# Guillaume-SOULIER/SOS-Radiative-Transfer

Measured on AMD Instinct MI355X. Metric: SOS columns/sec to 1e-4 convergence (Ntau=200, Nmu=128), higher is better.
Workload: dtype f64

## Files before the change

### sos-radiative-transfer_amd/csrc/jn_gemm.hip

```cpp
#include "jn_gemm_tile.hpp"

namespace sosrt {

namespace {

#ifndef SOSRT_DENSE_SLAB_RT
#define SOSRT_DENSE_SLAB_RT 1
#endif
constexpr int DENSE_SLAB_RT = SOSRT_DENSE_SLAB_RT;
#ifndef SOSRT_LIVE_TILE_MAJOR
#define SOSRT_LIVE_TILE_MAJOR 1
#endif
constexpr int DENSE_SLAB_ROWS = 16 * DENSE_SLAB_RT;

__device__ __forceinline__ void write_live_list(const GemmArgs& g) {
    __shared__ int s_cnt[4];
    const int tid = threadIdx.x, lane = tid & 63, wave = tid >> 6;
    int before = 0;
    for (int base = 0; base < g.B; base += 256) {
        const bool f = base + tid < g.B && g.active[g.col0 + base + tid] != 0;
        const unsigned long long mk = __ballot(f);
        if (lane == 0) s_cnt[wave] = __popcll(mk);
        __syncthreads();
        int pre = before, tot = 0;
        for (int w = 0; w < 4; ++w) {
            if (w < wave) pre += s_cnt[w];
            tot += s_cnt[w];
        }
        const int at = pre + __popcll(mk & ((1ull << lane) - 1));
        if (f && at < g.live_cap) g.live_list[at] = base + tid;
        before += tot;
        __syncthreads();
    }
    for (int i = before + tid; i < g.live_cap; i += 256) g.live_list[i] = -1;
}

template <bool SYM, bool ATM>
__device__ __forceinline__ void jn_gemm_dense(const GemmArgs& g, const AtmSets& at) {
    if (g.live_list && blockIdx.x == gridDim.x - 1) {
        write_live_list(g);
        return;
    }
    publish_live(g);
    __shared__ double sA[(SYM ? 2 : 1) * 16 * (GEMM_RT > 2 ? GEMM_RT : 2) * A_LD];
    __shared__ double sB[GEMM_KC * B_LD];
    __shared__ int s_any;
    const int tiles_main = (g.n_main + 16 * GEMM_RT - 1) / (16 * GEMM_RT);
    const int tiles_slab = (g.n_slab + DENSE_SLAB_ROWS - 1) / DENSE_SLAB_ROWS;
    const int tiles = tiles_main + tiles_slab;
    const int nct = (g.D + GEMM_BN - 1) / GEMM_BN;
    const int id = blockIdx.x;
    int tile = (id / (8 * nct)) * 8 + (id & 7);
    const int bn0 = ((id >> 3) % nct) * GEMM_BN;
    if (tile >= tiles) return;
    if (ATM || g.lr_rank >= 0) {
        if (tile >= tiles_slab) {
            lowrank_tile<false, ListRows, ATM>(g, ListRows{g.rows_main, g.n_main}, tile - tiles_slab, 16 * GEMM_RT, bn0, true, at);
            return;
        }
        tile += tiles_main;
    }
    if (tile < tiles_main) {
        gemm_tile<GEMM_RT, false, false, SYM>(g, sA, sB, &s_any, tile, bn0, ListRows{g.rows_main, g.n_main}, true);
    } else if (g.Wmix && g.slab_tile_group) {
        const int st = tile - tiles_main;
        gemm_tile<DENSE_SLAB_RT, false, false, SYM>(g, sA, sB, &s_any, st, bn0, ListRows{g.rows_slab, g.n_slab}, true,
                                                    g.Wmix + (size_t)g.slab_tile_group[st * DENSE_SLAB_ROWS / 32] * g.Dp * g.Wld);
    } else if (g.slab_tile_group) {
        const int st = tile - tiles_main;
        GemmArgs gs = g;
        gs.Wr = g.Wr + (size_t)g.slab_tile_group[st * DENSE_SLAB_ROWS / 32] * g.Dp * g.Wld;
        gemm_tile<DENSE_SLAB_RT, true, false, SYM>(gs, sA, sB, &s_any, st, bn0, ListRows{g.rows_slab, g.n_slab}, true);
    } else {
        gemm_tile<DENSE_SLAB_RT, true, false, SYM>(g, sA, sB, &s_any, tile - tiles_main, bn0, ListRows{g.rows_slab, g.n_slab}, true);
    }
}
template <bool SYM>
__global__ __launch_bounds__(256, GEMM_WPS) void k_jn_gemm(GemmArgs g) { jn_gemm_dense<SYM, false>(g, AtmSets()); }
__global__ __launch_bounds__(256, GEMM_WPS) void k_jn_gemm_atm(GemmArgs g, AtmSets at) { jn_gemm_dense<true, true>(g, at); }

template <int RT, bool DEEP, bool SYM, bool ATM = false>
__device__ __forceinline__ void gemm_live_columns(const GemmArgs& g, double* sA, double* sB, const AtmSets& at = AtmSets()) {
    __shared__ int s_w[4];
    __shared__ int s_col;
    const int tid = threadIdx.x, lane = tid & 63, wave = tid >> 6;
    const int ts = (g.max_slab + 16 * TAIL_RT_SLAB - 1) / (16 * TAIL_RT_SLAB);
    const int tm = (g.max_main + 16 * RT - 1) / (16 * RT);
    const int nct = (g.D + GEMM_BN - 1) / GEMM_BN;
    const int id = blockIdx.x;
    const int xq = (id / (8 * nct)) * 8 + (id & 7), bn0 = ((id >> 3) % nct) * GEMM_BN;
// ... 13 lines not shown
        if (lane == 0) s_w[wave] = __popcll(mk);
        __syncthreads();
        int pre = before, tot = 0;
        for (int w = 0; w < 4; ++w) {
            if (w < wave) pre += s_w[w];
            tot += s_w[w];
        }
        if (f && pre + __popcll(mk & ((2ull << lane) - 1)) == ci + 1) s_col = g.col0 + base + tid;
        before += tot;
        __syncthreads();
        if (before > ci) break;
    }
    const int b = s_col;
    if (g.live_list && xq < (SOSRT_LIVE_TILE_MAJOR ? (g.live_cap > 0 ? g.live_cap : 1) : 1 << 30) &&
        (SOSRT_LIVE_TILE_MAJOR || tt == 0) && bn0 == 0 && tid == 0 && ci < g.live_cap)
        g.live_list[ci] = b < 0 ? -1 : b - g.col0;
    if (b < 0) return;
    const int iu = g.idx_up ? g.idx_up[b] : 0;
    const int ns = g.idx_up ? g.idx_down[b] - iu + 1 : 0;
    if (tt < ts) {
        if (tt * 16 * TAIL_RT_SLAB >= ns) return;
        if (g.Wmix)
            gemm_tile<TAIL_RT_SLAB, false, DEEP, SYM>(g, sA, sB, nullptr, tt, bn0, ColumnRows{b * g.L, iu, ns, ns, true},
                                                      false, g.Wmix + (size_t)g.mix_group[b] * g.Dp * g.Wld);
        else if (g.mix_group) {
            GemmArgs gs = g;
            gs.Wr = g.Wr + (size_t)g.mix_group[b] * g.Dp * g.Wld;
            gemm_tile<TAIL_RT_SLAB, true, DEEP, SYM>(gs, sA, sB, nullptr, tt, bn0, ColumnRows{b * g.L, iu, ns, ns, true}, false);
        } else
            gemm_tile<TAIL_RT_SLAB, true, DEEP, SYM>(g, sA, sB, nullptr, tt, bn0, ColumnRows{b * g.L, iu, ns, ns, true}, false);
    } else {
        const int t2 = tt - ts;
        if (t2 * 16 * RT >= g.L - ns) return;
        if (ATM || g.lr_rank >= 0) lowrank_tile<false, ColumnRows, ATM>(g, ColumnRows{b * g.L, iu, ns, g.L - ns, false}, t2, 16 * RT, bn0, false, at);
        else gemm_tile<RT, false, DEEP, SYM>(g, sA, sB, nullptr, t2, bn0, ColumnRows{b * g.L, iu, ns, g.L - ns, false}, false);
    }
}

template <bool SYM>
__global__ __launch_bounds__(256, SYM ? 4 : GEMM_WPS) void k_jn_gemm_cols(GemmArgs g) {
    publish_live(g);
    __shared__ double sA[(SYM ? 2 : 1) * 16 * GEMM_RT * A_LD];
    __shared__ double sB[GEMM_KC * B_LD];
    gemm_live_columns<GEMM_RT, false, SYM>(g, sA, sB);
}
__global__ __launch_bounds__(256, 4) void k_jn_gemm_cols_atm(GemmArgs g, AtmSets at) {
    publish_live(g);
    __shared__ double sA[2 * 16 * GEMM_RT * A_LD];
    __shared__ double sB[GEMM_KC * B_LD];
    gemm_live_columns<GEMM_RT, false, true, true>(g, sA, sB, at);
}
constexpr bool kTailDeepSym = false;
constexpr int kTailWpsSym = 4;
template <bool SYM>
__global__ __launch_bounds__(256, SYM ? kTailWpsSym : 2) void k_jn_gemm_tail(GemmArgs g) {
    publish_live(g);
    __shared__ double sA[(SYM ? 2 : 1) * 16 * TAIL_RT * A_LD];
    __shared__ double sB[GEMM_KC * B_LD];
    gemm_live_columns<TAIL_RT, SYM ? kTailDeepSym : true, SYM>(g, sA, sB);
}
__global__ __launch_bounds__(256, kTailWpsSym) void k_jn_gemm_tail_atm(GemmArgs g, AtmSets at) {
    publish_live(g);
    __shared__ double sA[2 * 16 * TAIL_RT * A_LD];
    __shared__ double sB[GEMM_KC * B_LD];
    gemm_live_columns<TAIL_RT, kTailDeepSym, true, true>(g, sA, sB, at);
}
constexpr int kTailDeepCols = 32;
__global__ __launch_bounds__(256, 2) void k_jn_gemm_tail_deep(GemmArgs g) {
    publish_live(g);
    __shared__ double sA[2 * 16 * TAIL_RT * A_LD];
    __shared__ double sB[GEMM_KC * B_LD];
    gemm_live_columns<TAIL_RT, true, true>(g, sA, sB);
}
__global__ __launch_bounds__(256, 2) void k_jn_gemm_tail_deep_atm(GemmArgs g, AtmSets at) {
    publish_live(g);
    __shared__ double sA[2 * 16 * TAIL_RT * A_LD];
    __shared__ double sB[GEMM_KC * B_LD];
    gemm_live_columns<TAIL_RT, true, true, true>(g, sA, sB, at);
}

template <bool ATM>
__device__ __forceinline__ void jn_gemm_lone(const GemmArgs& g, const AtmSets& at) {
    extern __shared__ __attribute__((aligned(16))) double s_lone[];
    __shared__ int s_w[4];
    __shared__ int s_col[4];
    const int tid = threadIdx.x, lane = tid & 63, wave = tid >> 6;
    if (blockIdx.x == gridDim.x - 1) {
        if (g.host_pub && tid == 0) publish_live_now(g);
        return;
    }
    const int ts = (g.max_slab + 15) / 16, tm = (g.max_main + 15) / 16;
    const int nct = (g.D + GEMM_BN - 1) / GEMM_BN;
    const int id = blockIdx.x;
    const int xq = (id / (8 * nct)) * 8 + (id & 7), bn0 = ((id >> 3) % nct) * GEMM_BN;
    const int cap = g.live_cap > 0 ? g.live_cap : 1;
    const int tq = xq / cap, ci = xq % cap;
    if (tq >= ts + tm) return;
    const int tt = (ATM || g.lr_rank >= 0) ? tq : (tq < tm ? ts + tq : tq - tm);
    int fl = 0, iu_c = 0, id_c = -1, mg_c = 0;
    if (tid < g.B) {
        const int c = g.col0 + tid;
        fl = g.active[c];
        if (g.idx_up) {
            iu_c = g.idx_up[c]; id_c = g.idx_down[c];
            if (g.mix_group) mg_c = g.mix_group[c];
        }
    }
    LoneFrag f0, f1;
    const int nkb = (g.Ks >> 2) / LONE_KB;
    if (!ATM && tt >= ts && g.lr_rank < 0) {
// ... 14 lines not shown
            if (w < wave) pre += s_w[w];
            tot += s_w[w];
        }
        if (f && pre + __popcll(mk & ((2ull << lane) - 1)) == ci + 1) {
            s_col[0] = g.col0 + base + tid; s_col[1] = iu_c; s_col[2] = id_c - iu_c + 1; s_col[3] = mg_c;
        }
        before += tot;
        __syncthreads();
        if (before > ci || base + 256 >= g.B) break;
        fl = 0;
        if (base + 256 + tid < g.B) {
            const int c = g.col0 + base + 256 + tid;
            fl = g.active[c];
            if (g.idx_up) {
                iu_c = g.idx_up[c]; id_c = g.idx_down[c];
                if (g.mix_group) mg_c = g.mix_group[c];
            }
        }
    }
    const int b = s_col[0];
    if (g.live_list && tq == 0 && bn0 == 0 && tid == 0 && ci < g.live_cap) g.live_list[ci] = b < 0 ? -1 : b - g.col0;
    if (b < 0) return;
    const int iu = g.idx_up ? s_col[1] : 0, ns = g.idx_up ? s_col[2] : 0, mg = s_col[3];
    if (tt < ts) {
        if (tt * 16 >= ns) return;
        if (g.Wmix) gemm_tile_lone<false, false>(g, s_lone, tt, bn0, ColumnRows{b * g.L, iu, ns, ns, true}, f0, f1, g.Wmix + (size_t)mg * g.Dp * g.Wld);
        else if (g.mix_group) {
            GemmArgs gs = g;
            gs.Wr = g.Wr + (size_t)mg * g.Dp * g.Wld;
            gemm_tile_lone<true, false>(gs, s_lone, tt, bn0, ColumnRows{b * g.L, iu, ns, ns, true}, f0, f1);
        } else gemm_tile_lone<true, false>(g, s_lone, tt, bn0, ColumnRows{b * g.L, iu, ns, ns, true}, f0, f1);
    } else {
        if ((tt - ts) * 16 >= g.L - ns) return;
        if (ATM || g.lr_rank >= 0) lowrank_tile<false, ColumnRows, ATM>(g, ColumnRows{b * g.L, iu, ns, g.L - ns, false}, tt - ts, 16, bn0, false, at);
        else gemm_tile_lone<false, true>(g, s_lone, tt - ts, bn0, ColumnRows{b * g.L, iu, ns, g.L - ns, false}, f0, f1);
    }
}
__global__ __launch_bounds__(256, 1) void k_jn_gemm_lone(GemmArgs g) { jn_gemm_lone<false>(g, AtmSets()); }
__global__ __launch_bounds__(256, 1) void k_jn_gemm_lone_atm(GemmArgs g, AtmSets at) { jn_gemm_lone<true>(g, at); }

}

void launch_gemm_tail(hipStream_t s, const GemmArgs& a, int cols, bool small_tiles, bool regs, const AtmSets* at) {
    if (regs && a.sym) {
        const int ts = (a.max_slab + 15) / 16, tm = (a.max_main + 15) / 16;
        if (cols <= 0 || ts + tm <= 0) return;
        const int nct = (a.D + GEMM_BN - 1) / GEMM_BN;
        const int lds = 16 * (a.D + 2) * 8;
        static PerDeviceOnce big_lds;
        if (big_lds.first()) {
            hipFuncSetAttribute(reinterpret_cast<const void*>(k_jn_gemm_lone), hipFuncAttributeMaxDynamicSharedMemorySize, 150 * 1024);
            hipFuncSetAttribute(reinterpret_cast<const void*>(k_jn_gemm_lone_atm), hipFuncAttributeMaxDynamicSharedMemorySize, 150 * 1024);
        }
        const dim3 lgrid((unsigned)((cols * (ts + tm) + 7) / 8 * 8 * nct + 1));
        if (at) hipLaunchKernelGGL(k_jn_gemm_lone_atm, lgrid, dim3(256), (size_t)lds, s, a, *at);
        else hipLaunchKernelGGL(k_jn_gemm_lone, lgrid, dim3(256), (size_t)lds, s, a);
        return;
    }
    const int rt = small_tiles ? TAIL_RT : GEMM_RT;
    const int ts = (a.max_slab + 16 * TAIL_RT_SLAB - 1) / (16 * TAIL_RT_SLAB);
    const int tm = (a.max_main + 16 * rt - 1) / (16 * rt);
    if (cols <= 0 || ts + tm <= 0) return;
    const int nct = (a.D + GEMM_BN - 1) / GEMM_BN;
    dim3 grid((unsigned)((cols * (ts + tm) + 7) / 8 * 8 * nct));
    if (at) {
        if (small_tiles && cols <= kTailDeepCols) hipLaunchKernelGGL(k_jn_gemm_tail_deep_atm, grid, dim3(256), 0, s, a, *at);
        else if (small_tiles) hipLaunchKernelGGL(k_jn_gemm_tail_atm, grid, dim3(256), 0, s, a, *at);
// ... 69 lines not shown
                                                        double* __restrict__ out) {
    __shared__ double s_w[4], s_a[4];
    __shared__ int s_nan[4];
    const int q = blockIdx.y, tid = threadIdx.x;
    const double* Wq = W + (size_t)q * per;
    double wmax = 0, amax = 0;
    int nan = 0;
    const size_t n = (size_t)D * D;
    for (size_t e = (size_t)blockIdx.x * 256 + tid; e < n; e += (size_t)gridDim.x * 256) {
        const int k = (int)(e / D), m = (int)(e % D);
        const double x = Wq[(size_t)k * Wld + m], y = Wq[(size_t)(D - 1 - k) * Wld + (D - 1 - m)];
        const double ax = fabs(x), d = fabs(x - y);
        nan |= (ax != ax) || (d != d);
        wmax = fmax(wmax, ax); amax = fmax(amax, d);
    }
#pragma unroll
    for (int o = 32; o > 0; o >>= 1) {
        wmax = fmax(wmax, __shfl_xor(wmax, o, 64)); amax = fmax(amax, __shfl_xor(amax, o, 64));
        nan |= __shfl_xor(nan, o, 64);
    }
    if ((tid & 63) == 0) { s_w[tid >> 6] = wmax; s_a[tid >> 6] = amax; s_nan[tid >> 6] = nan; }
    __syncthreads();
    if (tid == 0) {
        for (int i = 1; i < 4; ++i) { wmax = fmax(wmax, s_w[i]); amax = fmax(amax, s_a[i]); nan |= s_nan[i]; }
        double* o = out + ((size_t)q * gridDim.x + blockIdx.x) * 2;
        o[0] = nan ? __builtin_nan("") : wmax;
        o[1] = nan ? __builtin_nan("") : amax;
    }
}
void launch_fold_asymmetry(hipStream_t s, int S, int nblk, int D, int Wld, size_t per, const double* W, double* out) {
    hipLaunchKernelGGL(k_fold_asymmetry, dim3((unsigned)nblk, (unsigned)S), dim3(256), 0, s, D, Wld, per, W, out);
}

void launch_gemm(hipStream_t s, const GemmArgs& a, const AtmSets* at) {
    const int tiles = (a.n_main + 16 * GEMM_RT - 1) / (16 * GEMM_RT) + (a.n_slab + DENSE_SLAB_ROWS - 1) / DENSE_SLAB_ROWS;
    if (tiles <= 0) return;
    const int nct = (a.D + GEMM_BN - 1) / GEMM_BN;
    dim3 grid((unsigned)((tiles + 7) / 8 * 8 * nct + (a.live_list ? 1 : 0)));
    if (at) hipLaunchKernelGGL(k_jn_gemm_atm, grid, dim3(256), (size_t)a.pad_lds, s, a, *at);
    else if (a.sym) hipLaunchKernelGGL(k_jn_gemm<true>, grid, dim3(256), (size_t)a.pad_lds, s, a);
    else hipLaunchKernelGGL(k_jn_gemm<false>, grid, dim3(256), (size_t)a.pad_lds, s, a);
}

__global__ void k_symfold(int nmat, int N, int D, int Dp, int Wld, const double* __restrict__ W, double* __restrict__ SA) {
    const size_t per = (size_t)Dp * Wld;
    const size_t i = (size_t)blockIdx.x * blockDim.x + threadIdx.x;
    if (i >= per * nmat) return;
    const size_t mat = i / per, r = i % per;
    const int k = (int)(r / Wld), c = (int)(r % Wld), Nh = Wld >> 1;
    const int m = c < Nh ? c : c - Nh;
    double out = 0.0;
    if (k < N && m < N) {
        const double* w = W + mat * per;
        const double p = w[(size_t)k * Wld + m], pf = w[(size_t)(D - 1 - k) * Wld + (D - 1 - m)];
        const double q = w[(size_t)(D - 1 - k) * Wld + m], qf = w[(size_t)k * Wld + (D - 1 - m)];
        out = c < Nh ? 0.25 * ((p + pf) + (q + qf)) : 0.25 * ((p + pf) - (q + qf));
    }
    SA[i] = out;
}
void launch_symfold(hipStream_t s, int nmat, int N, int D, int Dp, int Wld, const double* W, double* SA) {
    const size_t n = (size_t)Dp * Wld * nmat;
    hipLaunchKernelGGL(k_symfold, dim3((unsigned)((n + 255) / 256)), dim3(256), 0, s, nmat, N, D, Dp, Wld, W, SA);
}

}
```

### sos-radiative-transfer_amd/csrc/jn_gemm_tile.hpp

```cpp
#pragma once
#include "kernels.hpp"
#include "transport_util.hpp"

namespace sosrt {

namespace {

typedef double f64x4 __attribute__((ext_vector_type(4)));

constexpr int A_LD = GEMM_KC + 2;
constexpr int B_LD = GEMM_BN + 16;

struct ListRows {
    const int* rows;
    int n;
    __device__ int operator()(int lr) const { return lr < n ? (rows ? rows[lr] : lr) : -1; }
};
struct ColumnRows {
    int base, iu, ns, n;
    bool slab;
    __device__ int operator()(int lr) const {
        if (lr >= n) return -1;
        return base + (slab ? iu + lr : (lr < iu ? lr : lr + ns));
    }
// ... 310 lines not shown
        const double cf_ = pass_ ? cf_r : cf_a;                                                                   \
        const int k0_ = 4 * (b_ - pass_ * nkb) * LONE_KB + fk;                                                    \
        _Pragma("unroll") for (int q = 0; q < LONE_KB; ++q) {                                                     \
            const int k_ = k0_ + 4 * q;                                                                           \
            const bool ok_ = grow >= 0 && k_ < Nn;                                                                \
            const double a_ = arow[k_], m_ = arow[D - 1 - k_];                  \
            const double u_ = ok_ ? cf_ * (a_ + m_) : 0.0, v_ = ok_ ? cf_ * (a_ - m_) : 0.0;                      \
            accx = __builtin_amdgcn_mfma_f64_16x16x4f64(u_, F.s[q], accx, 0, 0, 0);                               \
            accy = __builtin_amdgcn_mfma_f64_16x16x4f64(v_, F.a[q], accy, 0, 0, 0);                               \
        }                                                                                                         \
    }
    for (int blk = 0; blk < nblk; blk += 2) {
        SOSRT_LONE_COMPUTE(f0, blk);
        SOSRT_LONE_LOAD(f0, blk + 2);
        if (blk + 1 < nblk) {
            SOSRT_LONE_COMPUTE(f1, blk + 1);
            SOSRT_LONE_LOAD(f1, blk + 3);
        }
    }
#undef SOSRT_LONE_LOAD
#undef SOSRT_LONE_COMPUTE
#pragma unroll
    for (int r = 0; r < 4; ++r) {
        const int gr = row_of(tile * 16 + 4 * r + fk);
        if (gr >= 0 && mcol < Nn) {
            const double x = accx[r], y = accy[r];
            g.C[(size_t)gr * D + mcol] = x + y;
            g.C[(size_t)gr * D + D - 1 - mcol] = x - y;
        }
    }
}

constexpr int LR_ROWS = 4;
template <bool COH, bool ATM = false>
__device__ __forceinline__ void lowrank_rows(const GemmArgs& g, const int (&rows)[LR_ROWS], int lane, const AtmSets& at = AtmSets()) {
    const int D = g.D, R = g.lr_rank;
    __amdgpu_buffer_rsrc_t rA[LR_ROWS], rC[LR_ROWS];
    double cf[LR_ROWS];
    int Ri[LR_ROWS];
    const double* __restrict__ Ui[LR_ROWS];
    const double* __restrict__ Vi[LR_ROWS];
#pragma unroll
    for (int i = 0; i < LR_ROWS; ++i) {
        const int r = rows[i] >= 0 ? rows[i] : rows[0];
        const int bytes = rows[i] >= 0 ? D * 8 : 0;
        rA[i] = make_rsrc(g.A + (size_t)r * D, bytes);
        rC[i] = make_rsrc(g.C + (size_t)r * D, bytes);
        cf[i] = rows[i] >= 0 ? g.ca[rows[i]] : 0.0;
        if constexpr (ATM) {
            const int st = __builtin_amdgcn_readfirstlane(at.col_atm[r / g.L]);
            Ri[i] = __builtin_amdgcn_readfirstlane(at.lr_ranks[st]);
            Ui[i] = g.lrU + (size_t)st * kLowRankMax * D;
            Vi[i] = g.lrV + (size_t)st * kLowRankMax * D;
        }
    }
    const double* __restrict__ U = g.lrU;
    const double* __restrict__ V = g.lrV;
    double m[LR_ROWS][kLowRankMax];
#pragma unroll
    for (int i = 0; i < LR_ROWS; ++i)
#pragma unroll
        for (int q = 0; q < kLowRankMax; ++q) m[i][q] = 0.0;
#pragma unroll 2
    for (int k = 2 * lane; k < D; k += 128) {
        double2 x[LR_ROWS];
#pragma unroll
        for (int i = 0; i < LR_ROWS; ++i) x[i] = bload2_aux<COH ? 16 : 0>(rA[i], k * 8, 0);
#pragma unroll
        for (int q = 0; q < kLowRankMax; ++q) {
            if constexpr (ATM) {
#pragma unroll
                for (int i = 0; i < LR_ROWS; ++i)
                    if (q < Ri[i]) {
                        const double2 u = *reinterpret_cast<const double2*>(Ui[i] + (size_t)q * D + k);
                        m[i][q] = __builtin_fma(x[i].y, u.y, __builtin_fma(x[i].x, u.x, m[i][q]));
                    }
            } else if (q < R) {
                const double2 u = *reinterpret_cast<const double2*>(U + (size_t)q * D + k);
#pragma unroll
                for (int i = 0; i < LR_ROWS; ++i) m[i][q] = __builtin_fma(x[i].y, u.y, __builtin_fma(x[i].x, u.x, m[i][q]));
            }
        }
    }
#pragma unroll
    for (int s = 32; s >= 1; s >>= 1)
#pragma unroll
        for (int q = 0; q < kLowRankMax; ++q) {
            if constexpr (ATM) {
#pragma unroll
                for (int i = 0; i < LR_ROWS; ++i)
                    if (q < Ri[i]) m[i][q] += __shfl_xor(m[i][q], s);
            } else if (q < R) {
#pragma unroll
                for (int i = 0; i < LR_ROWS; ++i) m[i][q] += __shfl_xor(m[i][q], s);
            }
        }
    if constexpr (!COH && !ATM) {
        if (g.mom) {
#pragma unroll
            for (int i = 0; i < LR_ROWS; ++i) {
                const int r = rows[i] >= 0 ? rows[i] : rows[0];
                const __amdgpu_buffer_rsrc_t rM = make_rsrc(g.mom + (size_t)r * kMomDoubles, rows[i] >= 0 ? kMomDoubles * 8 : 0);
                const double x = lane == 0 ? m[i][0] : (lane == 1 ? m[i][2] : (lane == 2 ? cf[i] : 0.0));
                const double y = lane == 0 ? m[i][1] : (lane == 1 ? m[i][3] : 0.0);
                bstore2(rM, lane * 16, 0, make_double2(x, y));
            }
            return;
        }
    }
#pragma unroll 2
    for (int k = 2 * lane; k < D; k += 128) {
        if constexpr (ATM) {
            double2 o[LR_ROWS];
#pragma unroll
            for (int i = 0; i < LR_ROWS; ++i) o[i] = make_double2(0.0, 0.0);
#pragma unroll
            for (int q = 0; q < kLowRankMax; ++q) {
#pragma unroll
                for (int i = 0; i < LR_ROWS; ++i)
                    if (q < Ri[i]) {
                        const double2 v = *reinterpret_cast<const double2*>(Vi[i] + (size_t)q * D + k);
                        o[i].x = __builtin_fma(m[i][q], v.x, o[i].x);
                        o[i].y = __builtin_fma(m[i][q], v.y, o[i].y);
                    }
            }
#pragma unroll
            for (int i = 0; i < LR_ROWS; ++i) bstore2_aux<COH ? 17 : 0>(rC[i], k * 8, 0, make_double2(cf[i] * o[i].x, cf[i] * o[i].y));
        } else {
            double vx[kLowRankMax], vy[kLowRankMax];
#pragma unroll
            for (int q = 0; q < kLowRankMax; ++q) {
                vx[q] = 0.0; vy[q] = 0.0;
                if (q < R) {
                    const double2 v = *reinterpret_cast<const double2*>(V + (size_t)q * D + k);
                    vx[q] = v.x; vy[q] = v.y;
                }
            }
#pragma unroll
            for (int i = 0; i < LR_ROWS; ++i)
                bstore2_aux<COH ? 17 : 0>(rC[i], k * 8, 0, make_double2(lr_expand(m[i], vx, R, cf[i]), lr_expand(m[i], vy, R, cf[i])));
        }
    }
}
template <bool COH, class RowOf, bool ATM = false>
__device__ __forceinline__ void lowrank_tile(const GemmArgs& g, RowOf row_of, int tile, int BM, int bn0, bool check_active,
                                             const AtmSets& at = AtmSets()) {
    const int nct = (g.D + GEMM_BN - 1) / GEMM_BN, ct = bn0 / GEMM_BN;
    const int lane = threadIdx.x & 63, wave = __builtin_amdgcn_readfirstlane(threadIdx.x) >> 6;
    const int per = (BM - ct + nct - 1) / nct;
    const bool chk = check_active && g.active && g.check_tiles;
    for (int j = LR_ROWS * wave; j < per; j += 4 * LR_ROWS) {
        int rows[LR_ROWS];
        int n = 0;
#pragma unroll
        for (int i = 0; i < LR_ROWS; ++i) {
            int r = j + i < per ? __builtin_amdgcn_readfirstlane(row_of(tile * BM + ct + nct * (j + i))) : -1;
            if (chk && r >= 0 && !g.active[r / g.L]) r = -1;
            rows[i] = r;
            n += r >= 0 ? 1 : 0;
        }
        if (n == 0) continue;
        if (rows[0] < 0)
#pragma unroll
            for (int i = 1; i < LR_ROWS; ++i)
                if (rows[i] >= 0) { rows[0] = rows[i]; rows[i] = -1; break; }
        lowrank_rows<COH, ATM>(g, rows, lane, at);
    }
}

constexpr int TAIL_RT_SLAB = 1;
constexpr int TAIL_RT = 2;

}
}
```

### sos-radiative-transfer_amd/csrc/kernels.hpp

```cpp
#pragma once
#include <hip/hip_runtime.h>

#include "plan.hpp"

namespace sosrt {

constexpr int kMaxZones = 8;
constexpr int kRingZones = 3;

struct alignas(16) ColDesc {
    int nz;
    int r0[kMaxZones];
    int r1[kMaxZones];
    int mix[kMaxZones];
    int nfix[kMaxZones];
    int fixtab[kMaxZones];
    int surface;
    int geom;
    double mu0, rho, T, tau_bottom;
    double wa;
    double wr[kMaxZones];
    double fa[kMaxZones];
    double fr[kMaxZones];
    double ca[kMaxZones];
// ... 128 lines not shown
    const double* Wa;
    const double* Wr;
    const double* ca;
    const double* cr;
    const int* rows_main;
    int n_main;
    const int* rows_slab;
    int n_slab;
    int D, Dp, Wld, L;
    double* C;
    const int* active;
    int B = 0;
    int col0 = 0;
    const int* idx_up = nullptr;
    const int* idx_down = nullptr;
    int max_main = 0, max_slab = 0;
    const double* Wmix = nullptr;
    const int* mix_group = nullptr;
    int pad_lds = 0;
    int* live_list = nullptr;
    int live_cap = 0;
    const int* slab_tile_group = nullptr;
    const int* nactive = nullptr;
    const int* need_small = nullptr;
    int* host_pub = nullptr;
    int tag = 0;
    int sym = 0;
    int Ks = 0;
    int check_tiles = 1;
    int lr_rank = -1;
    const double* lrU = nullptr;
    const double* lrV = nullptr;
    double* mom = nullptr;
};
struct AtmSets {
    const int* col_atm = nullptr;
    const int* lr_ranks = nullptr;
};
constexpr int kLowRankMax = 4;
constexpr int kMomDoubles = 8;

__device__ inline void publish_live_now(const GemmArgs& g) {
    const int live = __hip_atomic_load(g.nactive, __ATOMIC_RELAXED, __HIP_MEMORY_SCOPE_AGENT);
    int* slot = g.host_pub + 4 * (g.tag & 1);
    __hip_atomic_store(slot, live, __ATOMIC_RELAXED, __HIP_MEMORY_SCOPE_SYSTEM);
    __hip_atomic_store(slot + 2, g.need_small ? g.need_small[0] : 1, __ATOMIC_RELAXED, __HIP_MEMORY_SCOPE_SYSTEM);
    __hip_atomic_store(slot + 1, g.tag, __ATOMIC_RELEASE, __HIP_MEMORY_SCOPE_SYSTEM);
}
__device__ inline void publish_live(const GemmArgs& g) {
    if (g.host_pub && blockIdx.x == 0 && blockIdx.y == 0 && threadIdx.x == 0) publish_live_now(g);
}
struct PerDeviceOnce {
    bool seen[64] = {};
    bool first() {
        int d = 0;
        if (hipGetDevice(&d) != hipSuccess || d < 0 || d >= 64) return true;
        if (seen[d]) return false;
        seen[d] = true;
        return true;
    }
};
void launch_gemm(hipStream_t s, const GemmArgs& a, const AtmSets* at = nullptr);
struct OrderLoopArgs {
    TransportArgs t;
    GemmArgs gm;
    const double* in0;
    double* gbufP;
    double* gbufQ;
    double* bufP;
    double* bufQ;
    int order0;
    int kmax;
    int B, col0;
    int fixcap;
    int* sync;
    int* host_done;
    int tag;
    unsigned long long* log = nullptr;
    int astage = 0;
};
bool order_loop_ok(const Grid& g, bool split);
int order_loop_parts(const Grid& g, bool split);
hipError_t launch_order_loop(hipStream_t s, int grid, bool split, const OrderLoopArgs& p);
void launch_gemm_f32(hipStream_t s, const GemmArgs& a, const float* Wa32, const float* Wmix32);
void launch_to_float(hipStream_t s, size_t n, const double* src, float* dst);
void launch_wmix(hipStream_t s, size_t n, int ngroups, const double* Wa, const double* Wr, const double* ca, const double* cr,
                 double* Wmix, const int* gset = nullptr ,
                 const int* gatm = nullptr );
void launch_fold_sets(hipStream_t s, int S, int D, int Wld, size_t per, const double* w, const double* P, double* W);
void launch_fold_asymmetry(hipStream_t s, int S, int nblk, int D, int Wld, size_t per, const double* W, double* out);
void launch_symfold(hipStream_t s, int nmat, int N, int D, int Dp, int Wld, const double* W, double* SA);
void launch_gemm_tail(hipStream_t s, const GemmArgs& a, int cols, bool small_tiles, bool regs = false, const AtmSets* at = nullptr);
void launch_smallmu(hipStream_t s, const Grid& g, int B, const double* tau, const double* Jn, double* In,
                    const ColDesc* desc, const int* active);
void launch_transport(hipStream_t s, const Grid& g, int B, const double* tau, const double* Jn, double* In, double* I,
// ... 87 lines not shown
```

### sos-radiative-transfer_amd/csrc/solve.hip

```cpp
#include <hip/hip_runtime.h>

#include <algorithm>
#include <chrono>
#include <cstdio>
#include <cstdlib>
#include <mutex>
#include <string>
#include <vector>

#include "handle.hpp"

using namespace sosrt;

namespace {

int await_tag(sosrt_handle* h, volatile int* slot, int tag, int grp) {
    const auto t0 = std::chrono::steady_clock::now();
    auto next_query = t0 + std::chrono::milliseconds(20);
    for (unsigned it = 1;; ++it) {
        if (__atomic_load_n(&slot[1], __ATOMIC_ACQUIRE) == tag) return 0;
        if ((it & 0x3fff) == 0) {
            const auto now = std::chrono::steady_clock::now();
            if (grp >= 0 && now >= next_query) {
                next_query = now + std::chrono::milliseconds(20);
// ... 75 lines not shown
        ga.nactive = h->fld.d_nactive + pg; ga.need_small = h->fld.d_nactive + sosrt_handle::kMaxGroups;
        ga.host_pub = h->fld.h_pub + 8 * pg; ga.tag = o.pub_tag;
    }
    ga.check_tiles = o.all_live ? 0 : 1;
    AtmSets at;
    const AtmSets* atp = nullptr;
    if (h->cols.max_atm_used > 0) {
        at.col_atm = h->cols.d_colatm + (h->cols.nslab > 0 ? 0 : col0);
        at.lr_ranks = h->phase.d_lrranks.p;
        atp = &at;
    }
#ifdef SOSRT_DIAG
    if (ga.sym && h->gemm.diag_ks_mult > 1 && ga.Ks * h->gemm.diag_ks_mult <= h->g.Dp) ga.Ks *= h->gemm.diag_ks_mult;
#endif
    if (h->gemm.mode == SOSRT_CONTRACT_F32) {
        if (h->phase.w32_dirty) {
            prof_break(h);
            const size_t per = (size_t)h->g.Dp * h->g.Wld;
            launch_to_float(s, per, h->phase.d_Wa, h->phase.d_Wa32);
            if (h->cols.mix_groups > 0) launch_to_float(s, per * h->cols.mix_groups, h->cols.d_Wmix.p, h->cols.d_Wmix32.p);
            h->phase.w32_dirty = false;
        }
        prof_begin(h, SOSRT_K_GEMM, pg);
        launch_gemm_f32(s, ga, h->phase.d_Wa32, h->cols.d_Wmix32.p);
        prof_end(h, SOSRT_K_GEMM, pg);
        return;
    }
    prof_begin(h, SOSRT_K_GEMM, pg);
    if (live_tiles || (o.dense_live_cap > 0 && active && h->cols.nslab >= 0)) {
        ga.col0 = h->cols.nslab > 0 ? col0 : 0; ga.B = nb;
        ga.live_list = h->gemm.d_livelist + col0; ga.live_cap = live_tiles ? o.tail_cols : o.dense_live_cap;
    }
    if (live_tiles) launch_gemm_tail(s, ga, o.tail_cols, o.tail_cols <= h->gemm.gemm_small_cols, o.regs_tile, atp);
    else launch_gemm(s, ga, atp);
    prof_end(h, SOSRT_K_GEMM, pg);
}

struct SolveShape {
    bool ring_like = false;
    bool fast = false;
    int nzcap = kRingZones;
    int ring_mode = 1;
};
SolveShape solve_shape(const sosrt_handle* h, int max_nz) {
    SolveShape sh;
    sh.ring_like = h->tr.mode >= 2 && h->tr.ring_ok && (max_nz <= kRingZones || transport_ring_fits(h->g, max_nz));
    sh.fast = h->tr.mode >= 1 && h->tr.fast_ok && (max_nz <= kRingZones || sh.ring_like);
    sh.nzcap = max_nz > kRingZones ? max_nz : kRingZones;
    sh.ring_mode = (h->tr.mode >= 2 && h->tr.ring_ok) ? 3 : 1;
    return sh;
}
struct OrderInputs {
    int nb = 0;
    int known = 0;
    int surface = SOSRT_SURFACE_NONE;
    bool simple_zones = true;
    bool slabs_mixed = true;
    bool need_small = false;
    bool saving = false;
    int orders_left = 1 << 30;
    int cu_share = 0;
    bool atm_sets = false;
};
struct LaunchPlan {
    int tail_cols = 0;
    int live_cap = 0;
    int gemm = SOSRT_PLAN_GEMM_DENSE;
// ... 668 lines not shown
```

Before: 137,300.

## Stream low-rank GEMM rows through LDS-cached factors with pipelined loads

Adds a streaming low-rank path for the non-atmosphere case. Each wave handles a run of rows sized from the CU count. The U/V factors are staged in LDS, row loads are double-buffered against the FMA work, and the cross-lane reduction uses permlane/DPP instead of shfl_xor. The dense launch grid is resized to this run length, and tail/lone kernels also route low-rank tiles through the streaming variant. This is meant to cut redundant global reads of U/V and reduction latency, at the cost of extra LDS staging, more code paths, and a new dependency on correct CU-count plumbing.

```diff
diff --git a/sos-radiative-transfer_amd/csrc/jn_gemm.hip b/sos-radiative-transfer_amd/csrc/jn_gemm.hip
--- a/sos-radiative-transfer_amd/csrc/jn_gemm.hip
+++ b/sos-radiative-transfer_amd/csrc/jn_gemm.hip
@@ -42,20 +42,31 @@
         return;
     }
     publish_live(g);
-    __shared__ double sA[(SYM ? 2 : 1) * 16 * (GEMM_RT > 2 ? GEMM_RT : 2) * A_LD];
-    __shared__ double sB[GEMM_KC * B_LD];
+    constexpr int kSA = (SYM ? 2 : 1) * 16 * (GEMM_RT > 2 ? GEMM_RT : 2) * A_LD, kSB = GEMM_KC * B_LD;
+    __shared__ __attribute__((aligned(16))) double sA[kSA];
+    __shared__ __attribute__((aligned(16))) double sB[kSB];
     __shared__ int s_any;
     const int tiles_main = (g.n_main + 16 * GEMM_RT - 1) / (16 * GEMM_RT);
     const int tiles_slab = (g.n_slab + DENSE_SLAB_ROWS - 1) / DENSE_SLAB_ROWS;
     const int tiles = tiles_main + tiles_slab;
     const int nct = (g.D + GEMM_BN - 1) / GEMM_BN;
     const int id = blockIdx.x;
+    if (!ATM && g.lr_rank >= 0) {
+        const int slab_ids = (tiles_slab + 7) / 8 * 8 * nct;
+        if (id >= slab_ids) {
+            const int wave = __builtin_amdgcn_readfirstlane(threadIdx.x) >> 6;
+            const int rw = g.lr_run >> 2, first = (id - slab_ids) * g.lr_run + wave * rw;
+            lowrank_stream<true>(g, LrRun<ListRows>{ListRows{g.rows_main, g.n_main}, first, 1}, min(max(g.n_main - first, 0), rw), true,
+                           sA, kSA, sB, kSB);
+            return;
+        }
+    }
     int tile = (id / (8 * nct)) * 8 + (id & 7);
     const int bn0 = ((id >> 3) % nct) * GEMM_BN;
     if (tile >= tiles) return;
     if (ATM || g.lr_rank >= 0) {
         if (tile >= tiles_slab) {
-            lowrank_tile<false, ListRows, ATM>(g, ListRows{g.rows_main, g.n_main}, tile - tiles_slab, 16 * GEMM_RT, bn0, true, at);
+            if constexpr (ATM) lowrank_tile<false, ListRows, true>(g, ListRows{g.rows_main, g.n_main}, tile - tiles_slab, 16 * GEMM_RT, bn0, true, at);
             return;
         }
         tile += tiles_main;
@@ -135,7 +146,10 @@
     } else {
         const int t2 = tt - ts;
         if (t2 * 16 * RT >= g.L - ns) return;
-        if (ATM || g.lr_rank >= 0) lowrank_tile<false, ColumnRows, ATM>(g, ColumnRows{b * g.L, iu, ns, g.L - ns, false}, t2, 16 * RT, bn0, false, at);
+        if (ATM || (RT == GEMM_RT && g.lr_rank >= 0))
+            lowrank_tile<false, ColumnRows, ATM>(g, ColumnRows{b * g.L, iu, ns, g.L - ns, false}, t2, 16 * RT, bn0, false, at);
+        else if (g.lr_rank >= 0)
+            lowrank_stream_tile(g, ColumnRows{b * g.L, iu, ns, g.L - ns, false}, t2, 16 * RT, bn0, sA, (SYM ? 2 : 1) * 16 * RT * A_LD, sB, GEMM_KC * B_LD);
         else gemm_tile<RT, false, DEEP, SYM>(g, sA, sB, nullptr, t2, bn0, ColumnRows{b * g.L, iu, ns, g.L - ns, false}, false);
     }
 }
@@ -143,14 +157,14 @@
 template <bool SYM>
 __global__ __launch_bounds__(256, SYM ? 4 : GEMM_WPS) void k_jn_gemm_cols(GemmArgs g) {
     publish_live(g);
-    __shared__ double sA[(SYM ? 2 : 1) * 16 * GEMM_RT * A_LD];
-    __shared__ double sB[GEMM_KC * B_LD];
+    __shared__ __attribute__((aligned(16))) double sA[(SYM ? 2 : 1) * 16 * GEMM_RT * A_LD];
+    __shared__ __attribute__((aligned(16))) double sB[GEMM_KC * B_LD];
     gemm_live_columns<GEMM_RT, false, SYM>(g, sA, sB);
 }
 __global__ __launch_bounds__(256, 4) void k_jn_gemm_cols_atm(GemmArgs g, AtmSets at) {
     publish_live(g);
-    __shared__ double sA[2 * 16 * GEMM_RT * A_LD];
-    __shared__ double sB[GEMM_KC * B_LD];
+    __shared__ __attribute__((aligned(16))) double sA[2 * 16 * GEMM_RT * A_LD];
+    __shared__ __attribute__((aligned(16))) double sB[GEMM_KC * B_LD];
     gemm_live_columns<GEMM_RT, false, true, true>(g, sA, sB, at);
 }
 constexpr bool kTailDeepSym = false;
@@ -158,27 +172,27 @@
 template <bool SYM>
 __global__ __launch_bounds__(256, SYM ? kTailWpsSym : 2) void k_jn_gemm_tail(GemmArgs g) {
     publish_live(g);
-    __shared__ double sA[(SYM ? 2 : 1) * 16 * TAIL_RT * A_LD];
-    __shared__ double sB[GEMM_KC * B_LD];
+    __shared__ __attribute__((aligned(16))) double sA[(SYM ? 2 : 1) * 16 * TAIL_RT * A_LD];
+    __shared__ __attribute__((aligned(16))) double sB[GEMM_KC * B_LD];
     gemm_live_columns<TAIL_RT, SYM ? kTailDeepSym : true, SYM>(g, sA, sB);
 }
 __global__ __launch_bounds__(256, kTailWpsSym) void k_jn_gemm_tail_atm(GemmArgs g, AtmSets at) {
     publish_live(g);
-    __shared__ double sA[2 * 16 * TAIL_RT * A_LD];
-    __shared__ double sB[GEMM_KC * B_LD];
+    __shared__ __attribute__((aligned(16))) double sA[2 * 16 * TAIL_RT * A_LD];
+    __shared__ __attribute__((aligned(16))) double sB[GEMM_KC * B_LD];
     gemm_live_columns<TAIL_RT, kTailDeepSym, true, true>(g, sA, sB, at);
 }
 constexpr int kTailDeepCols = 32;
 __global__ __launch_bounds__(256, 2) void k_jn_gemm_tail_deep(GemmArgs g) {
     publish_live(g);
-    __shared__ double sA[2 * 16 * TAIL_RT * A_LD];
-    __shared__ double sB[GEMM_KC * B_LD];
+    __shared__ __attribute__((aligned(16))) double sA[2 * 16 * TAIL_RT * A_LD];
+    __shared__ __attribute__((aligned(16))) double sB[GEMM_KC * B_LD];
     gemm_live_columns<TAIL_RT, true, true>(g, sA, sB);
 }
 __global__ __launch_bounds__(256, 2) void k_jn_gemm_tail_deep_atm(GemmArgs g, AtmSets at) {
     publish_live(g);
-    __shared__ double sA[2 * 16 * TAIL_RT * A_LD];
-    __shared__ double sB[GEMM_KC * B_LD];
+    __shared__ __attribute__((aligned(16))) double sA[2 * 16 * TAIL_RT * A_LD];
+    __shared__ __attribute__((aligned(16))) double sB[GEMM_KC * B_LD];
     gemm_live_columns<TAIL_RT, true, true, true>(g, sA, sB, at);
 }
 
@@ -259,7 +273,9 @@
         } else gemm_tile_lone<true, false>(g, s_lone, tt, bn0, ColumnRows{b * g.L, iu, ns, ns, true}, f0, f1);
     } else {
         if ((tt - ts) * 16 >= g.L - ns) return;
-        if (ATM || g.lr_rank >= 0) lowrank_tile<false, ColumnRows, ATM>(g, ColumnRows{b * g.L, iu, ns, g.L - ns, false}, tt - ts, 16, bn0, false, at);
+        if (ATM) lowrank_tile<false, ColumnRows, true>(g, ColumnRows{b * g.L, iu, ns, g.L - ns, false}, tt - ts, 16, bn0, false, at);
+        else if (g.lr_rank >= 0)
+            lowrank_stream_tile(g, ColumnRows{b * g.L, iu, ns, g.L - ns, false}, tt - ts, 16, bn0, s_lone, 8 * (g.D + 2), s_lone + 8 * (g.D + 2), 8 * (g.D + 2));
         else gemm_tile_lone<false, true>(g, s_lone, tt - ts, bn0, ColumnRows{b * g.L, iu, ns, g.L - ns, false}, f0, f1);
     }
 }
@@ -395,11 +411,17 @@
     hipLaunchKernelGGL(k_fold_asymmetry, dim3((unsigned)nblk, (unsigned)S), dim3(256), 0, s, D, Wld, per, W, out);
 }
 
-void launch_gemm(hipStream_t s, const GemmArgs& a, const AtmSets* at) {
-    const int tiles = (a.n_main + 16 * GEMM_RT - 1) / (16 * GEMM_RT) + (a.n_slab + DENSE_SLAB_ROWS - 1) / DENSE_SLAB_ROWS;
+void launch_gemm(hipStream_t s, const GemmArgs& a_, const AtmSets* at, int cus) {
+    GemmArgs a = a_;
+    const int tiles_slab = (a.n_slab + DENSE_SLAB_ROWS - 1) / DENSE_SLAB_ROWS;
+    const int tiles = (a.n_main + 16 * GEMM_RT - 1) / (16 * GEMM_RT) + tiles_slab;
     if (tiles <= 0) return;
     const int nct = (a.D + GEMM_BN - 1) / GEMM_BN;
     dim3 grid((unsigned)((tiles + 7) / 8 * 8 * nct + (a.live_list ? 1 : 0)));
+    if (!at && a.lr_rank >= 0) {
+        a.lr_run = lr_stream_run(a.n_main, cus);
+        grid.x = (unsigned)((tiles_slab + 7) / 8 * 8 * nct + (a.n_main + a.lr_run - 1) / a.lr_run + (a.live_list ? 1 : 0));
+    }
     if (at) hipLaunchKernelGGL(k_jn_gemm_atm, grid, dim3(256), (size_t)a.pad_lds, s, a, *at);
     else if (a.sym) hipLaunchKernelGGL(k_jn_gemm<true>, grid, dim3(256), (size_t)a.pad_lds, s, a);
     else hipLaunchKernelGGL(k_jn_gemm<false>, grid, dim3(256), (size_t)a.pad_lds, s, a);
diff --git a/sos-radiative-transfer_amd/csrc/jn_gemm_tile.hpp b/sos-radiative-transfer_amd/csrc/jn_gemm_tile.hpp
--- a/sos-radiative-transfer_amd/csrc/jn_gemm_tile.hpp
+++ b/sos-radiative-transfer_amd/csrc/jn_gemm_tile.hpp
@@ -366,6 +366,40 @@
 }
 
 constexpr int LR_ROWS = 4;
+__device__ __forceinline__ void lr_accum(double& m, double2 x, double2 u) { m = __builtin_fma(x.y, u.y, __builtin_fma(x.x, u.x, m)); }
+template <int CTRL, int BANKS = 0xf>
+__device__ __forceinline__ double lr_dpp(double keep, double v) {
+    return __hiloint2double(__builtin_amdgcn_update_dpp(__double2hiint(keep), __double2hiint(v), CTRL, 0xf, BANKS, false),
+                            __builtin_amdgcn_update_dpp(__double2loint(keep), __double2loint(v), CTRL, 0xf, BANKS, false));
+}
+template <bool REG = true>
+__device__ __forceinline__ void lr_butterfly(double& m) {
+    if constexpr (!REG) {
+#pragma unroll
+        for (int s = 32; s >= 1; s >>= 1) m += __shfl_xor(m, s);
+        return;
+    }
+    {
+        const auto lo = __builtin_amdgcn_permlane32_swap(__double2loint(m), __double2loint(m), false, false);
+        const auto hi = __builtin_amdgcn_permlane32_swap(__double2hiint(m), __double2hiint(m), false, false);
+        m = __hiloint2double(hi[0], lo[0]) + __hiloint2double(hi[1], lo[1]);
+    }
+    {
+        const auto lo = __builtin_amdgcn_permlane16_swap(__double2loint(m), __double2loint(m), false, false);
+        const auto hi = __builtin_amdgcn_permlane16_swap(__double2hiint(m), __double2hiint(m), false, false);
+        m = __hiloint2double(hi[0], lo[0]) + __hiloint2double(hi[1], lo[1]);
+    }
+    m += lr_dpp<0x128>(m, m);
+    m += lr_dpp<0x114, 0xa>(lr_dpp<0x104, 0x5>(m, m), m);
+    m += lr_dpp<0x4e>(m, m);
+    m += lr_dpp<0xb1>(m, m);
+}
+__device__ __forceinline__ void lr_store_record(__amdgpu_buffer_rsrc_t rM, int lane, const double (&m)[kLowRankMax], double cf) {
+    const double x = lane == 0 ? m[0] : (lane == 1 ? m[2] : (lane == 2 ? cf : 0.0));
+    const double y = lane == 0 ? m[1] : (lane == 1 ? m[3] : 0.0);
+    bstore2(rM, lane * 16, 0, make_double2(x, y));
+}
+
 template <bool COH, bool ATM = false>
 __device__ __forceinline__ void lowrank_rows(const GemmArgs& g, const int (&rows)[LR_ROWS], int lane, const AtmSets& at = AtmSets()) {
     const int D = g.D, R = g.lr_rank;
@@ -405,39 +439,31 @@
             if constexpr (ATM) {
 #pragma unroll
                 for (int i = 0; i < LR_ROWS; ++i)
-                    if (q < Ri[i]) {
-                        const double2 u = *reinterpret_cast<const double2*>(Ui[i] + (size_t)q * D + k);
-                        m[i][q] = __builtin_fma(x[i].y, u.y, __builtin_fma(x[i].x, u.x, m[i][q]));
-                    }
+                    if (q < Ri[i]) lr_accum(m[i][q], x[i], *reinterpret_cast<const double2*>(Ui[i] + (size_t)q * D + k));
             } else if (q < R) {
                 const double2 u = *reinterpret_cast<const double2*>(U + (size_t)q * D + k);
 #pragma unroll
-                for (int i = 0; i < LR_ROWS; ++i) m[i][q] = __builtin_fma(x[i].y, u.y, __builtin_fma(x[i].x, u.x, m[i][q]));
-            }
-        }
-    }
-#pragma unroll
-    for (int s = 32; s >= 1; s >>= 1)
-#pragma unroll
-        for (int q = 0; q < kLowRankMax; ++q) {
-            if constexpr (ATM) {
-#pragma unroll
-                for (int i = 0; i < LR_ROWS; ++i)
-                    if (q < Ri[i]) m[i][q] += __shfl_xor(m[i][q], s);
-            } else if (q < R) {
-#pragma unroll
-                for (int i = 0; i < LR_ROWS; ++i) m[i][q] += __shfl_xor(m[i][q], s);
-            }
-        }
+                for (int i = 0; i < LR_ROWS; ++i) lr_accum(m[i][q], x[i], u);
+            }
+        }
+    }
+#pragma unroll
+    for (int q = 0; q < kLowRankMax; ++q) {
+        if constexpr (ATM) {
+#pragma unroll
+            for (int i = 0; i < LR_ROWS; ++i)
+                if (q < Ri[i]) lr_butterfly<false>(m[i][q]);
+        } else if (q < R) {
+#pragma unroll
+            for (int i = 0; i < LR_ROWS; ++i) lr_butterfly<!COH>(m[i][q]);
+        }
+    }
     if constexpr (!COH && !ATM) {
         if (g.mom) {
 #pragma unroll
             for (int i = 0; i < LR_ROWS; ++i) {
                 const int r = rows[i] >= 0 ? rows[i] : rows[0];
-                const __amdgpu_buffer_rsrc_t rM = make_rsrc(g.mom + (size_t)r * kMomDoubles, rows[i] >= 0 ? kMomDoubles * 8 : 0);
-                const double x = lane == 0 ? m[i][0] : (lane == 1 ? m[i][2] : (lane == 2 ? cf[i] : 0.0));
-                const double y = lane == 0 ? m[i][1] : (lane == 1 ? m[i][3] : 0.0);
-                bstore2(rM, lane * 16, 0, make_double2(x, y));
+                lr_store_record(make_rsrc(g.mom + (size_t)r * kMomDoubles, rows[i] >= 0 ? kMomDoubles * 8 : 0), lane, m[i], cf[i]);
             }
             return;
         }
@@ -502,6 +528,202 @@
     }
 }
 
+struct LrSet { double2 x[LR_ROWS][2]; };
+struct LrCursor {
+    unsigned long long todo;
+    int sel[LR_ROWS];
+    int c;
+};
+__device__ __forceinline__ void lr_next_batch(LrCursor& cu) {
+#pragma unroll
+    for (int i = 0; i < LR_ROWS; ++i) {
+        cu.sel[i] = cu.todo ? (int)__builtin_ctzll(cu.todo) : -1;
+        cu.todo &= cu.todo - 1;
+    }
+}
+template <bool WIDE>
+__device__ __forceinline__ void lr_issue(const GemmArgs& g, LrSet& X, LrCursor& cu, int rowv, int lane, int nc) {
+    if (!WIDE || cu.c == 0) lr_next_batch(cu);
+    const int k0 = 2 * lane + (WIDE ? 256 * cu.c : 0);
+    __builtin_amdgcn_sched_barrier(0);
+#pragma unroll
+    for (int i = 0; i < LR_ROWS; ++i) {
+        const int r = cu.sel[i] >= 0 ? __builtin_amdgcn_readlane(rowv, cu.sel[i]) : -1;
+        const __amdgpu_buffer_rsrc_t rA = make_rsrc(g.A + (size_t)(r >= 0 ? r : 0) * g.D, r >= 0 ? g.D * 8 : 0);
+#pragma unroll
+        for (int t = 0; t < 2; ++t) X.x[i][t] = bload2_aux<0>(rA, (k0 + 128 * t) * 8, 0);
+    }
+    __builtin_amdgcn_sched_barrier(0);
+    if (WIDE) cu.c = cu.c + 1 == nc ? 0 : cu.c + 1;
+}
+template <bool WIDE, int RT>
+__device__ __forceinline__ void lr_process(const GemmArgs& g, const LrSet& X, LrCursor& cu, double (&m)[LR_ROWS][RT], int rowv,
+                                           double cfv, int lane_, int nc, const double* sU, const double* sV, bool valid) {
+    const int D = g.D;
+    int lane = lane_;
+    asm volatile("" : "+v"(lane));
+    if (valid && (!WIDE || cu.c == 0)) lr_next_batch(cu);
+    if (!WIDE || (valid && cu.c == 0)) {
+#pragma unroll
+        for (int i = 0; i < LR_ROWS; ++i)
+#pragma unroll
+            for (int q = 0; q < RT; ++q) m[i][q] = 0.0;
+    }
+    const int k0 = 2 * lane + (WIDE ? 256 * cu.c : 0);
+    if (valid) {
+#pragma unroll
+        for (int t = 0; t < 2; ++t) {
+            const int k = k0 + 128 * t;
+            const bool in = k < D;
+#pragma unroll
+            for (int q = 0; q < RT; ++q) {
+                double2 u = *reinterpret_cast<const double2*>(sU + q * D + (in ? k : 0));
+                u.x = in ? u.x : -0.0; u.y = in ? u.y : -0.0;
+#pragma unroll
+                for (int i = 0; i < LR_ROWS; ++i) lr_accum(m[i][q], X.x[i][t], u);
+            }
+        }
+    }
+    const bool last = valid && (!WIDE || cu.c + 1 == nc);
+    if (WIDE && valid) cu.c = last ? 0 : cu.c + 1;
+    if (last) {
+#pragma unroll
+        for (int q = 0; q < RT; ++q) {
+#pragma unroll
+            for (int i = 0; i < LR_ROWS; ++i) lr_butterfly(m[i][q]);
+            if (RT > 2) __builtin_amdgcn_sched_barrier(0);
+        }
+    }
+    int row[LR_ROWS];
+    double cf[LR_ROWS];
+#pragma unroll
+    for (int i = 0; i < LR_ROWS; ++i) {
+        const bool have = last && cu.sel[i] >= 0;
+        const int l = have ? cu.sel[i] : 0;
+        row[i] = have ? __builtin_amdgcn_readlane(rowv, l) : -1;
+        cf[i] = __hiloint2double(__builtin_amdgcn_readlane(__double2hiint(cfv), l), __builtin_amdgcn_readlane(__double2loint(cfv), l));
+    }
+    if (g.mom) {
+#pragma unroll
+        for (int i = 0; i < LR_ROWS; ++i) {
+            const double M[kLowRankMax] = {m[i][0], RT > 1 ? m[i][RT > 1 ? 1 : 0] : 0.0, RT > 2 ? m[i][RT > 2 ? 2 : 0] : 0.0,
+                                           RT > 3 ? m[i][RT > 3 ? 3 : 0] : 0.0};
+            lr_store_record(make_rsrc(g.mom + (size_t)(row[i] >= 0 ? row[i] : 0) * kMomDoubles, row[i] >= 0 ? kMomDoubles * 8 : 0), lane,
+                            M, cf[i]);
+        }
+        return;
+    }
+    if (WIDE && !last) return;
+    __amdgpu_buffer_rsrc_t rC[LR_ROWS];
+#pragma unroll
+    for (int i = 0; i < LR_ROWS; ++i) rC[i] = make_rsrc(g.C + (size_t)(row[i] >= 0 ? row[i] : 0) * D, row[i] >= 0 ? D * 8 : 0);
+#pragma unroll 2
+    for (int k = 2 * lane; k < D; k += 128) {
+        double vx[kLowRankMax], vy[kLowRankMax];
+#pragma unroll
+        for (int q = 0; q < kLowRankMax; ++q) {
+            vx[q] = 0.0; vy[q] = 0.0;
+            if (q < RT) {
+                const double2 v = *reinterpret_cast<const double2*>(sV + q * D + k);
+                vx[q] = v.x; vy[q] = v.y;
+            }
+        }
+#pragma unroll
+        for (int i = 0; i < LR_ROWS; ++i) {
+            const double M[kLowRankMax] = {m[i][0], RT > 1 ? m[i][RT > 1 ? 1 : 0] : 0.0, RT > 2 ? m[i][RT > 2 ? 2 : 0] : 0.0,
+                                           RT > 3 ? m[i][RT > 3 ? 3 : 0] : 0.0};
+            bstore2_aux<0>(rC[i], k * 8, 0, make_double2(lr_expand(M, vx, RT, cf[i]), lr_expand(M, vy, RT, cf[i])));
+        }
+    }
+}
+template <bool WIDE, int RT, bool PIPE>
+__device__ __forceinline__ void lr_pipeline(const GemmArgs& g, unsigned long long todo, int rowv, double cfv, int lane,
+                                            const double* sU, const double* sV) {
+    const int nc = WIDE ? (g.D + 255) / 256 : 1;
+    const int nu = ((__popcll(todo) + LR_ROWS - 1) / LR_ROWS) * nc;
+    LrCursor ci{todo, {-1, -1, -1, -1}, 0}, cp = ci;
+    if constexpr (!PIPE) {
+        LrSet X;
+        double m1[LR_ROWS][RT];
+        for (int u = 0; u < nu; ++u) {
+            lr_issue<WIDE>(g, X, ci, rowv, lane, nc);
+            lr_process<WIDE, RT>(g, X, cp, m1, rowv, cfv, lane, nc, sU, sV, true);
+        }
+        return;
+    }
+    LrSet X0, X1;
+    double m[LR_ROWS][RT];
+    for (int u = 0; u <= nu; u += 2) {
+        lr_issue<WIDE>(g, X0, ci, rowv, lane, nc);
+        lr_process<WIDE, RT>(g, X1, cp, m, rowv, cfv, lane, nc, sU, sV, u > 0);
+        lr_issue<WIDE>(g, X1, ci, rowv, lane, nc);
+        lr_process<WIDE, RT>(g, X0, cp, m, rowv, cfv, lane, nc, sU, sV, true);
+    }
+}
+template <int RT, bool PIPE>
+__device__ __forceinline__ void lr_pipeline_width(const GemmArgs& g, unsigned long long todo, int rowv, double cfv, int lane,
+                                                  const double* sU, const double* sV) {
+    if (g.D <= 256) lr_pipeline<false, RT, PIPE>(g, todo, rowv, cfv, lane, sU, sV);
+    else lr_pipeline<true, RT, PIPE>(g, todo, rowv, cfv, lane, sU, sV);
+}
+template <class RowOf> struct LrRun {
+    RowOf row_of;
+    int first, stride;
+    __device__ int operator()(int i) const { return row_of(first + stride * i); }
+};
+template <bool PIPE, class RowAt>
+__device__ __forceinline__ void lowrank_stream(const GemmArgs& g, RowAt row_at, int n, bool check_active, double* sU, int capU,
+                                               double* sV, int capV) {
+    int tid_ = threadIdx.x;
+    asm volatile("" : "+v"(tid_));
+    const int tid = tid_, lane = tid & 63;
+    const int D = g.D, R = g.lr_rank;
+    const bool chk = check_active && g.active && g.check_tiles;
+    const bool lds = R > 0 && R * D <= capU && (g.mom || R * D <= capV);
+    int rowv = lane < n ? row_at(lane) : -1;
+    if (lds) {
+        const int n2 = R * D / 2;
+        for (int e = tid; e < n2; e += 256) {
+            reinterpret_cast<double2*>(sU)[e] = reinterpret_cast<const double2*>(g.lrU)[e];
+            if (!g.mom) reinterpret_cast<double2*>(sV)[e] = reinterpret_cast<const double2*>(g.lrV)[e];
+        }
+    }
+    int live = 1;
+    double cfv = 0.0;
+    if (rowv >= 0) {
+        if (chk) live = g.active[rowv / g.L];
+        cfv = g.ca[rowv];
+    }
+    const unsigned long long todo = __ballot(rowv >= 0 && live != 0);
+    if (lds) {
+        __syncthreads();
+        switch (R) {
+            case 1: lr_pipeline_width<1, PIPE>(g, todo, rowv, cfv, lane, sU, sV); break;
+            case 2: lr_pipeline_width<2, PIPE>(g, todo, rowv, cfv, lane, sU, sV); break;
+            case 3: lr_pipeline_width<3, PIPE>(g, todo, rowv, cfv, lane, sU, sV); break;
+            default: lr_pipeline_width<4, PIPE>(g, todo, rowv, cfv, lane, sU, sV); break;
+        }
+        return;
+    }
+    LrCursor cu{todo, {-1, -1, -1, -1}, 0};
+    while (cu.todo) {
+        lr_next_batch(cu);
+        int rows[LR_ROWS];
+#pragma unroll
+        for (int i = 0; i < LR_ROWS; ++i) rows[i] = cu.sel[i] >= 0 ? __builtin_amdgcn_readlane(rowv, cu.sel[i]) : -1;
+        lowrank_rows<false, false>(g, rows, lane);
+    }
+}
+template <class RowOf>
+__device__ __forceinline__ void lowrank_stream_tile(const GemmArgs& g, RowOf row_of, int tile, int BM, int bn0, double* sU, int capU,
+                                                    double* sV, int capV) {
+    const int nct = (g.D + GEMM_BN - 1) / GEMM_BN, ct = bn0 / GEMM_BN;
+    const int wave = __builtin_amdgcn_readfirstlane(threadIdx.x) >> 6;
+    const int per = (BM - ct + nct - 1) / nct;
+    const int rw = (per + 4 * LR_ROWS - 1) / (4 * LR_ROWS) * LR_ROWS;
+    lowrank_stream<false>(g, LrRun<RowOf>{row_of, tile * BM + ct + nct * wave * rw, nct}, min(max(per - wave * rw, 0), rw), false, sU, capU, sV, capV);
+}
+
 constexpr int TAIL_RT_SLAB = 1;
 constexpr int TAIL_RT = 2;
 
diff --git a/sos-radiative-transfer_amd/csrc/kernels.hpp b/sos-radiative-transfer_amd/csrc/kernels.hpp
--- a/sos-radiative-transfer_amd/csrc/kernels.hpp
+++ b/sos-radiative-transfer_amd/csrc/kernels.hpp
@@ -184,12 +184,22 @@
     const double* lrU = nullptr;
     const double* lrV = nullptr;
     double* mom = nullptr;
+    int lr_run = 0;
 };
 struct AtmSets {
     const int* col_atm = nullptr;
     const int* lr_ranks = nullptr;
 };
 constexpr int kLowRankMax = 4;
+#ifndef SOSRT_LR_STREAM_ROUNDS
+#define SOSRT_LR_STREAM_ROUNDS 2
+#endif
+constexpr int kLrStreamRounds = SOSRT_LR_STREAM_ROUNDS;
+inline int lr_stream_run(int n_main, int cus) {
+    const long long wgs = (long long)(cus > 0 ? cus : 256) * 4 * kLrStreamRounds;
+    const long long run = ((n_main + wgs - 1) / wgs + 15) / 16 * 16;
+    return (int)(run < 16 ? 16 : (run > 256 ? 256 : run));
+}
 constexpr int kMomDoubles = 8;
 
 __device__ inline void publish_live_now(const GemmArgs& g) {
@@ -212,7 +222,7 @@
         return true;
     }
 };
-void launch_gemm(hipStream_t s, const GemmArgs& a, const AtmSets* at = nullptr);
+void launch_gemm(hipStream_t s, const GemmArgs& a, const AtmSets* at = nullptr, int cus = 0 );
 struct OrderLoopArgs {
     TransportArgs t;
     GemmArgs gm;
diff --git a/sos-radiative-transfer_amd/csrc/solve.hip b/sos-radiative-transfer_amd/csrc/solve.hip
--- a/sos-radiative-transfer_amd/csrc/solve.hip
+++ b/sos-radiative-transfer_amd/csrc/solve.hip
@@ -131,7 +131,7 @@
         ga.live_list = h->gemm.d_livelist + col0; ga.live_cap = live_tiles ? o.tail_cols : o.dense_live_cap;
     }
     if (live_tiles) launch_gemm_tail(s, ga, o.tail_cols, o.tail_cols <= h->gemm.gemm_small_cols, o.regs_tile, atp);
-    else launch_gemm(s, ga, atp);
+    else launch_gemm(s, ga, atp, h->cu_count);
     prof_end(h, SOSRT_K_GEMM, pg);
 }
 
```

After: 145,600 (median of 6 runs). 6.1% higher.
